# TensorHusker/Butterfly

Hardware: AMD Instinct MI355X
Metric: tokens/sec (node) + p50 latency, Llama-3-70B split across 1/2/4/8 MI355X (higher is better)
Workload: dtype bf16; 1 GPU; model=Llama-3-70B, global_batch=64, seq_len=1024, parallelism=single, hipgraph=True, kv_cache_dtype=bfloat16, async_decode=True, mixed=True, prefix_caching=True

## Files before the change

### butterfly_amd/ops/__init__.py

```python
from __future__ import annotations

import os
import threading
from typing import Optional
from pathlib import Path

import torch

from . import reference as ref
from .reference import SILU_INTERLEAVE, interleave_gate_up, rope_tables, split_gate_up

_LIB_PATH = Path(__file__).resolve().parent.parent / "_C.so"
_loaded = False
_load_error: str | None = None

EPILOGUES = {"none": 0, "bias": 1, "silu": 2}
DECODE_PART_TOKENS = 0


def load_library(path: str | os.PathLike | None = None) -> bool:
    global _loaded, _load_error
    if _loaded:
        return True
    p = Path(path) if path else Path(os.environ.get("BFLY_KERNEL_LIB") or _LIB_PATH)
# ... 528 lines not shown
        torch.ops.bfly.w8_scale_cols(y, scale, out, epi)
    return out


def linear_silu_gate(x, w, gates, e0: int, num_local: int, packed=None):
    if isinstance(x, RowNormed) or not _gpu(x):
        h = linear(x, w, epilogue="silu")
        return moe_gate_scale_(h, gates, e0, num_local)
    out = _empty(x.shape[0], w.shape[0] // 2, dtype=x.dtype, device=x.device)
    if packed is not None and torch.ops.bfly.gemm_packed(x, packed, out, 3, None, 0.0, gates, e0, num_local) > 0:
        return out
    torch.ops.bfly.gemm_silu_gate(x, w, out, gates, e0, num_local)
    return out


def gemm_plan(M: int, N: int, K: int) -> dict:
    load_library()
    k, mt, nt, bm, bn, sk, wk = torch.ops.bfly.gemm_plan(M, N, K)
    return {"kind": ("skinny", "tile", "big", "dec", "big8", "mid8", "big4", "mid4")[k], "mt": mt, "nt": nt, "wk": wk, "bm": bm, "bn": bn,
            "splitk": sk}


def attn_prefill(q, k, v, cu_seqlens, max_seqlen: int, scale: float, causal: bool = True,
                 out=None, cu_seqlens_k=None, return_lse: bool = False):
    if not _gpu(q):
        return ref.attn_prefill(q, k, v, cu_seqlens, max_seqlen, scale, causal, out, cu_seqlens_k, return_lse)
    if out is None:
        out = _empty(q.shape, dtype=q.dtype, device=q.device)
    lse = _empty(q.shape[0], q.shape[1], dtype=torch.float32, device=q.device) if return_lse else None
    torch.ops.bfly.attn_prefill(q, k, v, cu_seqlens, max_seqlen, scale, causal, out, cu_seqlens_k, lse)
    return (out, lse) if return_lse else out


def attn_prefill_paged(q, k_cache, v_cache, tables, cu_q, positions, max_q: int, scale: float, out=None):
    if not _gpu(q):
# ... 136 lines not shown
```

### butterfly_amd/utils/flags.py

```python
from __future__ import annotations

import os
from dataclasses import dataclass
from typing import Any, Callable


@dataclass(frozen=True)
class Flag:
    name: str
    default: Any
    parse: Callable[[str], Any]
    help: str


def _bool(s: str) -> bool:
    return s.strip().lower() in ("1", "true", "yes", "on")


FLAGS: dict[str, Flag] = {}


def define(name: str, default, parse, help: str) -> Flag:
    f = Flag(name, default, parse, help)
    FLAGS[name] = f
# ... 12 lines not shown
define("BFLY_CUSTOM_AR", True, _bool, "use the one-shot IPC all-reduce kernel (self-tested at start-up, "
       "RCCL otherwise) for small TP all-reduces")
define("BFLY_CUSTOM_AR_MAX_BYTES", 8 << 20, int, "largest all-reduce (bytes) routed to the IPC kernel")
define("BFLY_CUSTOM_AR_AUTOTUNE", True, _bool, "time the IPC all-reduce (one- / two-shot) against RCCL at start-up "
       "and route each message size to the faster one (0: the fixed BFLY_CUSTOM_AR_* thresholds)")
define("BFLY_AR_BUTTERFLY", "", str, "\"W@lo:hi[,...]\": all-reduces of lo..hi bytes over a group of W ranks (bare "
       "\"lo:hi\": any power-of-two group) run as the butterfly "
       "(recursive halving + doubling over point-to-point transfers, parallel/butterfly.py), outside graph capture; set by "
       "the start-up probe only where it measured faster than RCCL and the IPC kernel (empty = never)")
define("BFLY_PROBE_BUTTERFLY", False, _bool, "the start-up comm probe also times the butterfly all-reduce (and may "
       "route sizes to it through BFLY_AR_BUTTERFLY)")
define("BFLY_CUSTOM_AR_2SHOT_BYTES", 512 << 10, int, "IPC all-reduces of at least this many bytes over 4 or 8 "
       "ranks run as reduce-scatter + all-gather (2S/W bytes per link instead of S; 0 = always one-shot)")
define("BFLY_GEMM_TUNED", True, _bool, "consult the measured GEMM plan table (0: heuristic plans only; read by the kernel library)")
define("BFLY_GEMM_NT_WEIGHTS", True, _bool, "stream decode GEMM weights with the non-temporal policy (read by the kernel library)")
define("BFLY_GEMM_PLAN", "", str, "force GEMM plans for whole-model A/B runs: \"N,K,Mbucket:kind,mt,nt,wk,bm,bn,sk;...\" "
       "(read by the kernel library)")
define("BFLY_ATTN_XCD", 1, int, "prefill attention: XCD-aware item walk (0: plain order; read by the kernel library)")
define("BFLY_ATTN_TRACE", "", str, "set: the prefill attention kernel stamps its item phases into the LSE buffer "
       "instead of writing results (tools/attn_trace.py; read by the kernel library)")
define("BFLY_KERNEL_LIB", "", str, "path of another build of the kernel library (same-box A/B runs of kernel changes)")
define("BFLY_LOG_JSON", False, _bool, "emit log records as one JSON object per line")
define("BFLY_RESTART", 0, int, "restart attempt of this job (set by `launch --max-restarts`; 0 = first run)")
define("BFLY_ATTN_PAGED_LDS", True, _bool, "paged-prefix prefill attention: the LDS-staged kernel for chunks of "
       "several sequences (0: the register kernel everywhere; read by the kernel library)")
define("BFLY_DEFER_REDUCE", True, _bool, "fuse split-K GEMM reduces into the consuming rope / add+rmsnorm kernels")
define("BFLY_NORM_ROWSCALE", True, _bool, "decode add+RMSNorm split over (row, 1024-column) workgroups that write x * g "
       "and partial sums of squares; the consuming QKV / gate-up GEMM applies the 1/rms row scale in its epilogue "
       "(tp == 1, batches <= BFLY_NORM_ROWSCALE_MAX_ROWS; 0: one-workgroup-per-row add+RMSNorm)")
define("BFLY_NORM_ROWSCALE_MAX_ROWS", 256, int, "largest batch that takes the row-split add+RMSNorm")
# ... 83 lines not shown
```

### csrc/bindings/ops.cpp

```cpp
#include <ATen/ATen.h>
#include <ATen/hip/impl/HIPStreamMasqueradingAsCUDA.h>
#include <c10/core/DeviceGuard.h>
#include <torch/library.h>

#include "bfly_kernels.h"

namespace {

using at::Tensor;

inline hipStream_t cur_stream() { return at::hip::getCurrentHIPStreamMasqueradingAsCUDA().stream(); }

inline bfly::bf16* bf(const Tensor& t) { return reinterpret_cast<bfly::bf16*>(t.data_ptr()); }

#define CHECK_GPU(t) TORCH_CHECK((t).is_cuda(), #t " must be a GPU tensor")
#define CHECK_BF16(t) TORCH_CHECK((t).scalar_type() == at::kBFloat16, #t " must be bf16")
#define CHECK_INNER(t) TORCH_CHECK((t).stride(-1) == 1, #t " must have unit inner stride")
#define CHECK_ALIGN16(t) \
  TORCH_CHECK(reinterpret_cast<uintptr_t>((t).data_ptr()) % 16 == 0, #t " must be 16-B aligned")
#define CHECK_KV(k, v)                                                                          \
  TORCH_CHECK(((k).scalar_type() == at::kBFloat16 || (k).scalar_type() == at::kFloat8_e4m3fn) && \
                  (v).scalar_type() == (k).scalar_type(),                                       \
              "KV caches must both be bf16 or both float8_e4m3fn")
#define CHECK_I32(t) TORCH_CHECK((t).scalar_type() == at::kInt, #t " must be int32")
// ... 517 lines not shown
    ws = workspace->data_ptr<float>();
    ws_bytes = workspace->numel() * sizeof(float);
  }
  c10::DeviceGuard g(x.device());
  const int rc = bfly::launch_gemm_w8(bf(x), x.stride(0), u8(code), scale.data_ptr<float>(), M, N, K, (int)epilogue,
                                      bf(out), out.stride(0), ws, ws_bytes, cur_stream(), any_m, (int)force_sk);
  TORCH_CHECK(rc == 0, "gemm_w8: shape / plan not taken by the native kernel M=", M, " N=", N, " K=", K,
              " (rc=", rc, ")");
}

int64_t gemm_packed_check(int64_t M, int64_t N, int64_t K, int64_t epilogue) {
  return bfly::launch_gemm_packed(nullptr, 0, nullptr, (int)M, (int)N, (int)K, (int)epilogue, nullptr, 0, nullptr,
                                  nullptr, true);
}

void gemm_with_plan(const Tensor& x, const Tensor& w, Tensor& out, std::vector<int64_t> plan,
                    int64_t epilogue, const c10::optional<Tensor>& workspace,
                    const c10::optional<Tensor>& bias) {
  CHECK_GPU(x); CHECK_BF16(x); CHECK_BF16(w); CHECK_BF16(out);
  TORCH_CHECK(x.dim() == 2 && w.dim() == 2 && out.dim() == 2 && plan.size() == 7, "gemm_with_plan: args");
  CHECK_INNER(x); CHECK_INNER(w); CHECK_INNER(out);
  const int M = x.size(0), K = x.size(1), N = w.size(0);
  TORCH_CHECK(w.size(1) == K, "gemm_with_plan: K mismatch");
  const int nout = epilogue == bfly::EPI_SILU ? N / 2 : N;
  TORCH_CHECK(out.size(0) == M && out.size(1) == nout, "gemm_with_plan: out shape");
  bfly::GemmPlan p{};
  p.kind = plan[0]; p.mt = plan[1]; p.nt = plan[2]; p.wk = plan[3]; p.bm = plan[4]; p.bn = plan[5]; p.sk = plan[6];
  float* ws = nullptr;
  size_t ws_bytes = 0;
  if (workspace.has_value()) {
    ws = reinterpret_cast<float*>(workspace->data_ptr());
    ws_bytes = workspace->numel() * workspace->element_size();
  }
  const bfly::bf16* bp = nullptr;
  if (bias.has_value()) {
    TORCH_CHECK(epilogue == bfly::EPI_BIAS && bias->numel() == N && bias->is_contiguous(), "gemm_with_plan: bias");
    CHECK_BF16(*bias);
    bp = bf(*bias);
  }
  TORCH_CHECK(epilogue != bfly::EPI_BIAS || bp != nullptr, "gemm_with_plan: bias epilogue needs a bias");
  c10::DeviceGuard g(x.device());
  const int rc = bfly::launch_gemm_plan(p, bf(x), x.stride(0), bf(w), w.stride(0), M, N, K, epilogue,
                                        bp, bf(out), out.stride(0), ws, ws_bytes, cur_stream());
  TORCH_CHECK(rc == 0, "gemm_with_plan: plan rejected (rc=", rc, ")");
}

int64_t gemm_deferred(const Tensor& x, const Tensor& w, Tensor& out, Tensor& workspace) {
  CHECK_GPU(x); CHECK_BF16(x); CHECK_BF16(w); CHECK_BF16(out);
  TORCH_CHECK(x.dim() == 2 && w.dim() == 2 && out.dim() == 2, "gemm_deferred: 2-D operands");
  CHECK_INNER(x); CHECK_INNER(w); CHECK_INNER(out);
  CHECK_ALIGN16(x); CHECK_ALIGN16(w);
  const int M = x.size(0), K = x.size(1), N = w.size(0);
  TORCH_CHECK(w.size(1) == K && K % 64 == 0 && N % 128 == 0, "gemm_deferred: shape");
  TORCH_CHECK(x.stride(0) % 8 == 0 && w.stride(0) % 8 == 0, "gemm_deferred: row strides % 8");
  TORCH_CHECK(out.size(0) == M && out.size(1) == N && out.is_contiguous(), "gemm_deferred: out");
  TORCH_CHECK(workspace.scalar_type() == at::kFloat && workspace.is_contiguous(), "gemm_deferred: workspace");
  c10::DeviceGuard g(x.device());
  const int rc = bfly::launch_gemm_deferred(bf(x), x.stride(0), bf(w), w.stride(0), M, N, K, bf(out),
// ... 663 lines not shown
  m.def("gemm_packed(Tensor x, Tensor wp, Tensor(a!) out, int epilogue, Tensor? ssp=None, float eps=0.0, "
        "Tensor? gates=None, int e0=0, int num_local=1, Tensor(b!)? workspace=None, bool defer=False) -> int");
  m.def("gemm_packed_check(int M, int N, int K, int epilogue) -> int", &gemm_packed_check);
  m.def("quant_fp8_rows(Tensor w, Tensor(a!) code, Tensor(b!) scale) -> ()");
  m.def("dequant_fp8(Tensor code, Tensor? scale, Tensor(a!) out) -> ()");
  m.def("w8_scale_cols(Tensor y, Tensor scale, Tensor(a!) out, int epilogue) -> ()");
  m.def("gemm_w8(Tensor x, Tensor code, Tensor scale, Tensor(a!) out, int epilogue, Tensor(b!)? workspace, "
        "bool any_m=False, int force_sk=0) -> ()");
  m.def("gemm_w8_check(int M, int N, int K, int epilogue) -> int",
        [](int64_t M, int64_t N, int64_t K, int64_t e) -> int64_t { return bfly::gemm_w8_check(M, N, K, e); });
  m.def("gemm_w8_splitk(int M, int N, int K, int epilogue) -> int",
        [](int64_t M, int64_t N, int64_t K, int64_t e) -> int64_t { return bfly::gemm_w8_splitk(M, N, K, e); });
  m.def("gemm_w8_workspace_size(int M, int N, int K) -> int",
        [](int64_t M, int64_t N, int64_t K) -> int64_t { return (int64_t)bfly::gemm_w8_workspace_bytes(M, N, K); });
  m.def("gemm_with_plan(Tensor x, Tensor w, Tensor(a!) out, int[] plan, int epilogue, Tensor(b!)? workspace, "
        "Tensor? bias=None) -> ()");
  m.def("gemm_workspace_size(int M, int N, int K) -> int", &gemm_workspace_size);
  m.def("gemm_plan(int M, int N, int K) -> int[]", &gemm_plan);
  m.def("gemm_check(int M, int N, int K, int epilogue) -> int",
        [](int64_t M, int64_t N, int64_t K, int64_t e) -> int64_t { return bfly::gemm_check(M, N, K, e); });
  m.def("attn_decode_splits(int max_ctx, int part_tokens) -> int", &attn_decode_splits);
  m.def("attn_decode_part_tokens(int B, int Hkv, int max_ctx) -> int", &attn_decode_part_tokens);
  m.def("attn_decode(Tensor q, Tensor k_cache, Tensor v_cache, Tensor block_tables, Tensor ctx_lens, "
        "float scale, int max_ctx, int part_tokens, Tensor(a!) out, Tensor(b!)? part_o, "
        "Tensor(c!)? part_ml) -> ()");
  m.def("moe_route(Tensor x, Tensor wr, int top_k, Tensor(a!) gates, Tensor(b!) topk_ids, Tensor(c!) topk_w) -> ()");
  m.def("moe_gate_scale(Tensor(a!) h, Tensor gates, int e0, int num_local) -> ()");
  m.def("moe_max_tiles(int tk, int num_local, int bm=64) -> int", &moe_max_tiles);
  m.def("moe_align(Tensor topk_ids, int e0, int num_local, Tensor(a!) rows, Tensor(b!) slot_of, Tensor(c!) tiles, "
        "Tensor(d!) count, int bm=64, Tensor? bcnt=None, int bcap=0) -> ()");
  m.def("moe_grouped_gemm(Tensor x, Tensor w, Tensor(a!) out, Tensor? rows, Tensor tiles, Tensor count, int w_estride, "
// ... 99 lines not shown
```

### csrc/include/bfly_kernels.h

```cpp
#pragma once
#include <hip/hip_runtime.h>
#include <stddef.h>
#include <stdint.h>

namespace bfly {

typedef __bf16 bf16;

enum GemmEpilogue { EPI_NONE = 0, EPI_BIAS = 1, EPI_SILU = 2, EPI_SILU_GATE = 3 };

struct RowScale {
  const float* ss;
  int chunks;
  float inv_dim, eps;
  const float* gate = nullptr;
  int gld = 0, ge0 = 0, gF = 0;
};

struct GemmPlan {
  int kind;
  int mt, nt;
  int wk;
  int bm, bn;
  int sk;
// ... 51 lines not shown
constexpr int kLogprobsMaxChunks = 64;
inline int logprobs_chunks(int V) { return (V + kLogprobsChunk - 1) / kLogprobsChunk; }
inline size_t logprobs_workspace_words(long rows, int V, int n) {
  return (size_t)rows * logprobs_chunks(V) * (2 + n);
}
void launch_logprobs_partial(const bf16* logits, long row_stride, int rows, int V, int vstart,
                             const int* ids, int n, uint64_t* workspace, float* record,
                             hipStream_t stream);
void launch_logprobs_merge(const float* records, int tp, int rows, int n, float* chosen_lp,
                           int* top_ids, float* top_lp, hipStream_t stream);

GemmPlan plan_gemm(int M, int N, int K);
size_t gemm_workspace_bytes(int M, int N, int K);
int launch_gemm_plan(const GemmPlan& p, const bf16* X, long ldx, const bf16* W, long ldw, int M,
                     int N, int K, int epi, const bf16* bias, bf16* out, long ldo, float* ws,
                     size_t ws_bytes, hipStream_t stream);
int gemm_check(int M, int N, int K, int epi);
int gemm_rowscale_check(int M, int N, int K, int epi);
int launch_gemm_deferred(const bf16* X, long ldx, const bf16* W, long ldw, int M, int N, int K,
                         bf16* out, long ldo, float* ws, size_t ws_bytes, hipStream_t stream,
                         const RowScale* rs = nullptr);
size_t gemm_slab_offset_floats();
void launch_splitk_reduce(const float* part, int sk, int M, int N, bf16* out, long ldo,
                          hipStream_t stream);
int launch_gemm(const bf16* X, long ldx, const bf16* W, long ldw, int M, int N, int K, int epi,
                const bf16* bias, bf16* out, long ldo, float* ws, size_t ws_bytes,
                hipStream_t stream, const RowScale* rs = nullptr);
int launch_gemm_packed(const bf16* X, long ldx, const bf16* Wp, int M, int N, int K, int epi, bf16* out,
                       long ldo, hipStream_t stream, const RowScale* rs = nullptr, bool dry = false,
                       float* ws = nullptr, size_t ws_bytes = 0, bool defer = false);
int launch_gemm_silu_gate(const bf16* X, long ldx, const bf16* W, long ldw, int M, int N, int K,
// ... 101 lines not shown
```

### csrc/kernels/gemm.hip

```cpp
#include "bfly_common.h"

#include <cstdio>
#include <string>
#include <vector>
#include "bfly_kernels.h"
#include "bfly_kv.h"

namespace bfly {

typedef __attribute__((address_space(3))) void* lds_ptr_t;

__constant__ int g_tile_w_nt = 1;
typedef __attribute__((address_space(1))) void* gbl_ptr_t;

__device__ __forceinline__ void store_out(bf16* out, long ldo, int m, int n, float v) {
  out[(long)m * ldo + n] = f2bf(v);
}

__device__ __forceinline__ void store_out4(bf16* out, long ldo, int m, int n, f32x4 v, bool vec) {
  bf16* p = out + (long)m * ldo + n;
  if (vec) {
    bf16x4 o;
#pragma unroll
    for (int r = 0; r < 4; ++r) o[r] = f2bf(v[r]);
// ... 183 lines not shown
    else
      __builtin_amdgcn_global_load_lds((gbl_ptr_t)g, (lds_ptr_t)(lds + blk * 1024), 16, 0, 0);
  }
}

template <int N>
__device__ __forceinline__ void vm_wait() {
  asm volatile("s_waitcnt vmcnt(%0)" ::"n"(N) : "memory");
}

__device__ __forceinline__ bf16x8 lds_frag(const char* lds, int row, int chunk) {
  const int slot = chunk ^ ((row >> 1) & 7);
  return *reinterpret_cast<const bf16x8*>(lds + row * 128 + slot * 16);
}

template <int TI, int TJ>
__device__ __forceinline__ void tile_epilogue(const f32x4 (&acc)[TI][TJ], int mw, int nw, int lane,
                                              int M, int N, int epi, const bf16* __restrict__ bias,
                                              bf16* __restrict__ out, long ldo, float* __restrict__ pslab,
                                              int m0, const RowScale& rsc) {
  const int lr = lane & 15, lc = 4 * (lane >> 4);
  const auto rs = slab_rsrc(pslab, pslab ? (long)(M - m0) * N * 4 : 0);
  const bool vec = (ldo & 3) == 0 && (reinterpret_cast<uintptr_t>(out) & 7) == 0;
  float sc[TI];
#pragma unroll
  for (int i = 0; i < TI; ++i) sc[i] = 1.f;
  if (rsc.ss != nullptr) {
    const int q = lane >> 4, nc = rsc.chunks;
#pragma unroll
    for (int i = 0; i < TI; ++i) {
      const int m = min(mw + 16 * i + lr, M - 1);
// ... 14 lines not shown
    }
  }
#pragma unroll
  for (int i = 0; i < TI; ++i) {
    const int m = mw + 16 * i + lr;
    if (m >= M) continue;
#pragma unroll
    for (int j = 0; j < TJ; ++j) {
      const int n = nw + 16 * j + lc;
      if (pslab) {
        store_slab4(rs, ((m - m0) * N + n) * 4, acc[i][j] * sc[i]);
      } else if (epi == EPI_SILU || epi == EPI_SILU_GATE) {
        if constexpr (TJ % 2 == 0) {
          if (j & 1) continue;
          f32x4 h;
#pragma unroll
          for (int r = 0; r < 4; ++r) h[r] = silu(acc[i][j][r] * sc[i]) * (acc[i][j + 1][r] * sc[i]);
          const int f = nw / 2 + 16 * (j / 2) + lc;
          if (epi == EPI_SILU_GATE) {
            const float g = rsc.gate[(long)m * rsc.gld + rsc.ge0 + f / rsc.gF];
#pragma unroll
            for (int r = 0; r < 4; ++r) h[r] = bf2f(f2bf(h[r])) * g;
          }
          store_out4(out, ldo, m, f, h, vec);
        }
      } else {
        f32x4 v = acc[i][j] * sc[i];
        if (epi == EPI_BIAS) {
#pragma unroll
          for (int r = 0; r < 4; ++r) v[r] += bf2f(bias[n + r]);
        }
        store_out4(out, ldo, m, n, v, vec);
// ... 82 lines not shown
    for (int ks = 0; ks < 2; ++ks) {
      bf16x8 af[TI], bfr[TJ];
#pragma unroll
      for (int i = 0; i < TI; ++i) af[i] = lds_frag(As, wm * WM + 16 * i + (lane & 15), ks * 4 + (lane >> 4));
#pragma unroll
      for (int j = 0; j < TJ; ++j) bfr[j] = lds_frag(Bs, wn * WN + 16 * j + (lane & 15), ks * 4 + (lane >> 4));
#pragma unroll
      for (int i = 0; i < TI; ++i)
#pragma unroll
        for (int j = 0; j < TJ; ++j) acc[i][j] = mfma16(bfr[j], af[i], acc[i][j]);
    }
    if (++buf == STAGES) buf = 0;
  }
  tile_epilogue<TI, TJ>(acc, m0 + wm * WM, n0 + wn * WN, lane, M, N, epi, bias, out, ldo,
                        part ? part + (long)ksplit * m_slab * N + (long)m0 * N : nullptr, m0, rsc);
}

template <int ROWS, int NW>
constexpr int ring_loads() { return (ROWS / 8 + NW - 1) / NW; }

template <int ROWS, int NW>
__device__ __forceinline__ void ring_stage(const bf16* __restrict__ src, long ld, int row0, int row_max,
                                           int k0, char* lds, int wid, int lane, bool nt) {
  constexpr int kBlocks = ROWS / 8;
#pragma unroll
  for (int i = 0; i < ring_loads<ROWS, NW>(); ++i) {
    int blk = i * NW + wid;
    if (kBlocks % NW != 0) blk %= kBlocks;
    const int row = blk * 8 + (lane >> 3);
    const int chunk = (lane & 7) ^ ((row >> 1) & 7);
// ... 772 lines not shown
  init_nt_policy();
  const int tiles = ((M + BM - 1) / BM) * (N / BN);
  const size_t lds = (size_t)STAGES * (BM + BN) * kBK * 2;
  const dim3 grid(tiles, sk);
  static bool attr_set = false;
  if (!attr_set && lds > 65536) {
    hipFuncSetAttribute(reinterpret_cast<const void*>(&gemm_tile_kernel<BM, BN, WMW, STAGES, false, PACKW>),
                        hipFuncAttributeMaxDynamicSharedMemorySize, (int)lds);
    attr_set = true;
  }
  gemm_tile_kernel<BM, BN, WMW, STAGES, false, PACKW><<<grid, kTileThreads, lds, stream>>>(
      X, ldx, W, PACKW ? (long)K : ldw, M, N, K, epi, bias, out, ldo, sk > 1 ? splitk_part(ws) : nullptr,
      nullptr, nullptr, nullptr, 0, rsc);
}

template <int BM, int BN, int NWM, int NWN, int SW>
static void run_dec(const bf16* X, long ldx, const bf16* W, long ldw, int M, int N, int K,
                    int epi, const bf16* bias, bf16* out, long ldo, float* ws, int sk,
                    hipStream_t stream, const RowScale& rsc) {
  init_nt_policy();
  const int tiles = ((M + BM - 1) / BM) * (N / BN);
  constexpr size_t lds = (size_t)(3 * BM + SW * BN) * kBK * 2;
  static_assert(lds <= 160 * 1024, "decode GEMM rings exceed the 160 KiB LDS");
  static bool attr_set = false;
  if (!attr_set && lds > 65536) {
    hipFuncSetAttribute(reinterpret_cast<const void*>(&gemm_dec_kernel<BM, BN, NWM, NWN, SW>),
                        hipFuncAttributeMaxDynamicSharedMemorySize, (int)lds);
    attr_set = true;
  }
  const dim3 grid(tiles, sk);
// ... 87 lines not shown
    size_t pos = 0;
    while (pos < s.size()) {
      size_t end = s.find(';', pos);
      if (end == std::string::npos) end = s.size();
      PlanOverride o{};
      if (sscanf(s.substr(pos, end - pos).c_str(), "%d,%d,%d:%d,%d,%d,%d,%d,%d,%d", &o.N, &o.K, &o.M, &o.p.kind,
                 &o.p.mt, &o.p.nt, &o.p.wk, &o.p.bm, &o.p.bn, &o.p.sk) == 10)
        out.push_back(o);
      pos = end + 1;
    }
    return out;
  }();
  return v;
}

GemmPlan plan_gemm(int M, int N, int K) {
  if (!plan_overrides().empty()) {
    static const int kB[] = {1, 16, 32, 64, 128, 256, 512};
    int bucket = 0;
    for (int b : kB)
      if (b >= M) { bucket = b; break; }
    for (const PlanOverride& o : plan_overrides())
      if (o.N == N && o.K == K && o.M == bucket) return o.p;
  }
  if (!tuned_enabled()) return plan_gemm_heuristic(M, N, K);
  static const int kBuckets[] = {1, 16, 32, 64, 128, 256, 512};
  int bucket = 0;
  for (int b : kBuckets)
    if (b >= M) { bucket = b; break; }
  if (bucket == 0) return plan_gemm_heuristic(M, N, K);
  for (const TunedPlan& t : kTuned)
    if (t.N == N && t.K == K && t.M == bucket)
      return t.kind == 4 ? GemmPlan{6, 0, 0, 0, 256, 256, t.sk}
                         : GemmPlan{t.kind, t.mt, t.nt, t.wk, t.bm, t.bn, t.sk};
  return plan_gemm_heuristic(M, N, K);
}

static GemmPlan plan_gemm_heuristic(int M, int N, int K) {
  GemmPlan p{};
  const int target = 448;
  const bool skinny_ok = K % 128 == 0 && N % 128 == 0;
  if (skinny_ok && (M <= 4 || (M <= 64 && K <= 1024))) {
    p.kind = 0;
    p.mt = (M + 15) / 16;
    const bool long_k = K > 4096;
    p.nt = M <= 4 ? (long_k ? 4 : 2) : 2;
    p.wk = long_k ? 2 : 4;
    const int blocks = N / (16 * p.nt * (4 / p.wk));
    int sk = 1;
    const int nchunks = K / 128;
// ... 29 lines not shown
static size_t plan_ws_bytes(const GemmPlan& p, int M, int N) {
  return p.sk > 1 ? kCounterBytes + (size_t)p.sk * M * N * sizeof(float) : 0;
}

size_t gemm_workspace_bytes(int M, int N, int K) {
  const size_t a = plan_ws_bytes(plan_gemm(M, N, K), M, N);
  const size_t b = plan_ws_bytes(plan_gemm_heuristic(M, N, K), M, N);
  return a > b ? a : b;
}

static int run_plan(const GemmPlan& p, const bf16* X, long ldx, const bf16* W, long ldw, int M,
                    int N, int K, int epi, const bf16* bias, bf16* out, long ldo, float* ws,
                    hipStream_t stream, bool dry = false, bool defer = false,
                    const RowScale* rs = nullptr, bool packed = false) {
  const RowScale rsc = rs ? *rs : RowScale{nullptr, 0, 0.f, 0.f};
  if (rs != nullptr && p.kind != 1 && p.kind != 3 && p.kind != 5 && p.kind != 7) return -4;
  if (epi == EPI_SILU_GATE && (p.kind != 1 || p.sk != 1)) return -4;
  if (packed && p.kind != 5 && p.kind != 7) return -5;
  if (p.kind == 4) {
    if (N % 256 != 0 || K % 64 != 0 || K / 64 < 2 * p.sk) return -1;
    if (!dry) run_big8(X, ldx, W, ldw, M, N, K, epi, bias, out, ldo, ws, p.sk, stream);
  } else if (p.kind == 7) {
    if (N % p.bn != 0 || K % 64 != 0 || K / 64 < p.sk) return -1;
    bool done = false;
#define MID4_CASE(BM_, BN_, SA_, SB_)                                                               \
  if (!done && p.bm == BM_ && p.bn == BN_ && p.mt == SA_ && p.nt == SB_) {                          \
    if (!dry && packed) run_mid4<BM_, BN_, SA_, SB_, true>(X, ldx, W, ldw, M, N, K, epi, bias, out, ldo, ws, p.sk, stream, rsc); \
    else if (!dry) run_mid4<BM_, BN_, SA_, SB_>(X, ldx, W, ldw, M, N, K, epi, bias, out, ldo, ws, p.sk, stream, rsc); \
    done = true;                                                                                   \
  }
    MID4_CASE(128, 128, 4, 6) MID4_CASE(128, 128, 3, 7) MID4_CASE(128, 128, 2, 8)
    MID4_CASE(256, 128, 3, 4) MID4_CASE(256, 128, 2, 6) MID4_CASE(128, 256, 4, 3) MID4_CASE(128, 256, 2, 4)
#undef MID4_CASE
// ... 41 lines not shown
    if (N % (16 * p.nt * (4 / p.wk)) != 0) return -1;
    if (epi == EPI_SILU && p.nt % 2 != 0) return -1;
    if (p.sk > 1 && N / (16 * p.nt * (4 / p.wk)) > kSplitCounters) return -1;
    bool done = false;
#define SK_CASE(MT_, NT_, WK_)                                                                   \
  if (!done && p.mt == MT_ && p.nt == NT_ && p.wk == WK_) {                                       \
    if (!dry) run_skinny<MT_, NT_, WK_>(X, ldx, W, ldw, M, N, K, epi, bias, out, ldo, ws, p.sk, stream); \
    done = true;                                                                                  \
  }
#define SK_WK(MT_, NT_) SK_CASE(MT_, NT_, 1) SK_CASE(MT_, NT_, 2) SK_CASE(MT_, NT_, 4)
    SK_WK(1, 1) SK_WK(1, 2) SK_WK(1, 4) SK_WK(2, 1) SK_WK(2, 2) SK_WK(2, 4)
    SK_WK(3, 2) SK_WK(4, 1) SK_WK(4, 2) SK_WK(4, 4)
#undef SK_WK
#undef SK_CASE
    if (!done) return -2;
  } else if (p.kind == 1 && p.nt == 1) {
    if (N % 256 != 0 || K % 64 != 0 || (p.bm != 16 && p.bm != 32 && p.bm != 64) || (p.bn != 128 && p.bn != 256) ||
        K / kBK < p.sk)
      return -1;
    if (p.sk > 1 && (long)((M + p.bm - 1) / p.bm) * (N / p.bn) > kSplitCounters) return -1;
    bool done = false;
    const int st = p.mt > 0 ? p.mt : 2;
#define TLP_CASE(BM_, BN_, WMW_, ST_)                                                                 \
  if (!done && p.bm == BM_ && p.bn == BN_ && p.wk == WMW_ && st == ST_) {                             \
    if (!dry) run_tile<BM_, BN_, WMW_, ST_, true>(X, ldx, W, ldw, M, N, K, epi, bias, out, ldo, ws, p.sk, stream, rsc); \
    done = true;                                                                                      \
  }
#define TLP_ST(BM_, BN_, WMW_) TLP_CASE(BM_, BN_, WMW_, 2) TLP_CASE(BM_, BN_, WMW_, 3) TLP_CASE(BM_, BN_, WMW_, 4)
    TLP_ST(16, 128, 1) TLP_ST(16, 256, 1) TLP_ST(32, 128, 1) TLP_ST(32, 256, 1)
    TLP_ST(64, 128, 1) TLP_ST(64, 128, 2) TLP_ST(64, 256, 1) TLP_ST(64, 256, 2)
#undef TLP_ST
// ... 19 lines not shown
    if (!done) return -2;
  }
  if (p.sk > 1 && !dry && !defer) {
    const int nout = epi == EPI_SILU ? N / 2 : N;
    long total = (long)M * nout;
    int grid = (int)((total + 255) / 256);
    if (grid > 4096) grid = 4096;
    gemm_splitk_reduce_kernel<<<grid, 256, 0, stream>>>(splitk_part(ws), p.sk, M, N, epi, bias,
                                                         out, ldo);
  }
  return 0;
}

int launch_gemm_plan(const GemmPlan& p, const bf16* X, long ldx, const bf16* W, long ldw, int M,
                     int N, int K, int epi, const bf16* bias, bf16* out, long ldo, float* ws,
                     size_t ws_bytes, hipStream_t stream) {
  if (M <= 0) return 0;
  if (p.sk > 1 && (ws == nullptr || ws_bytes < kCounterBytes + (size_t)p.sk * M * N * sizeof(float)))
    return -3;
  return run_plan(p, X, ldx, W, ldw, M, N, K, epi, bias, out, ldo, ws, stream);
}

static GemmPlan select_plan(int M, int N, int K, int epi) {
  GemmPlan p = plan_gemm(M, N, K);
  if (run_plan(p, nullptr, 0, nullptr, 0, M, N, K, epi, nullptr, nullptr, 0, nullptr, nullptr, true) != 0)
    p = plan_gemm_heuristic(M, N, K);
  return p;
}

int gemm_rowscale_check(int M, int N, int K, int epi) {
  if (M <= 0) return 0;
  const RowScale probe{nullptr, 0, 0.f, 0.f};
  return run_plan(select_plan(M, N, K, epi), nullptr, 0, nullptr, 0, M, N, K, epi, nullptr, nullptr, 0,
                  nullptr, nullptr, true, false, &probe);
}
// ... 84 lines not shown
}

int launch_gemm(const bf16* X, long ldx, const bf16* W, long ldw, int M, int N, int K, int epi,
                const bf16* bias, bf16* out, long ldo, float* ws, size_t ws_bytes,
                hipStream_t stream, const RowScale* rs) {
  if (M <= 0) return 0;
  GemmPlan p = select_plan(M, N, K, epi);
  if (p.sk > 1 && (ws == nullptr || ws_bytes < kCounterBytes + (size_t)p.sk * M * N * sizeof(float)))
    p.sk = 1;
  return run_plan(p, X, ldx, W, ldw, M, N, K, epi, bias, out, ldo, ws, stream, false, false, rs);
}

struct PackedTuned { int N, K, M; GemmPlan p; };
static const PackedTuned kPackedTuned[] = {
    {8192, 8192, 64, {1, 3, 1, 2, 64, 128, 4}},
    {4096, 4096, 1, {-1, 0, 0, 0, 0, 0, 0}},
    {4096, 4096, 16, {-1, 0, 0, 0, 0, 0, 0}},
    {4096, 4096, 32, {-1, 0, 0, 0, 0, 0, 0}},
    {4096, 4096, 64, {-1, 0, 0, 0, 0, 0, 0}},
};

int launch_gemm_packed(const bf16* X, long ldx, const bf16* Wp, int M, int N, int K, int epi, bf16* out,
                       long ldo, hipStream_t stream, const RowScale* rs, bool dry, float* ws, size_t ws_bytes,
                       bool defer) {
  if (M <= 0) return dry ? 0 : 1;
  if (N % 256 != 0 || K % 64 != 0) return -1;
  GemmPlan p = plan_gemm(M, N, K);
  if (tuned_enabled() && plan_overrides().empty() && epi != EPI_SILU_GATE) {
    static const int kB[] = {1, 16, 32, 64, 128, 256, 512};
    int bucket = 0;
    for (int b : kB)
      if (b >= M) { bucket = b; break; }
    for (const PackedTuned& t : kPackedTuned)
      if (t.N == N && t.K == K && t.M == bucket) {
        if (t.p.kind < 0) return -2;
        if (run_plan(t.p, nullptr, 0, nullptr, 0, M, N, K, epi, nullptr, nullptr, 0, nullptr, nullptr, true) == 0)
          p = t.p;
        break;
      }
  }
  if (epi != EPI_SILU_GATE &&
      run_plan(p, nullptr, 0, nullptr, 0, M, N, K, epi, nullptr, nullptr, 0, nullptr, nullptr, true) != 0)
    p = plan_gemm_heuristic(M, N, K);
  if (epi == EPI_SILU_GATE &&
      run_plan(p, nullptr, 0, nullptr, 0, M, N, K, epi, nullptr, nullptr, 0, nullptr, nullptr, true) != 0) {
    const int bm = M <= 16 ? 16 : M <= 32 ? 32 : M <= 64 ? 64 : 128;
    p = GemmPlan{1, 3, 0, bm <= 32 ? 1 : 2, bm, 128, 1};
  }
  const bool mid = (p.kind == 5 || p.kind == 7) && (p.bn == 128 || p.bn == 256);
  if (!mid && (p.kind != 1 || (p.bm != 16 && p.bm != 32 && p.bm != 64) || (p.bn != 128 && p.bn != 256))) return -2;
  if (!dry && p.sk > 1 && (ws == nullptr || ws_bytes < kCounterBytes + (size_t)p.sk * M * N * sizeof(float)))
    return -3;
  if (!mid) p.nt = 1;
  if (dry)
    return run_plan(p, nullptr, 0, nullptr, 0, M, N, K, epi, nullptr, nullptr, 0, nullptr, nullptr, true, false,
                    nullptr, mid);
  const bool d = defer && p.sk > 1;
  const int rc = run_plan(p, X, ldx, Wp, K, M, N, K, epi, nullptr, out, ldo, ws, stream, false, d, rs, mid);
  if (rc != 0) return rc;
  return d ? p.sk : 1;
}

int launch_gemm_silu_gate(const bf16* X, long ldx, const bf16* W, long ldw, int M, int N, int K,
                          bf16* out, long ldo, const float* gates, int gld, int ge0, int gF,
                          hipStream_t stream) {
  if (M <= 0) return 0;
  if (gates == nullptr || gF <= 0 || gF % 16 != 0 || (N / 2) % gF != 0) return -5;
  GemmPlan p = plan_gemm(M, N, K);
  if (run_plan(p, nullptr, 0, nullptr, 0, M, N, K, EPI_SILU_GATE, nullptr, nullptr, 0, nullptr, nullptr, true) != 0) {
    const int bm = M <= 16 ? 16 : M <= 32 ? 32 : M <= 64 ? 64 : 128;
    p = GemmPlan{1, 3, 0, bm <= 32 ? 1 : 2, bm, 128, 1};
  }
  RowScale rs{nullptr, 0, 0.f, 0.f};
// ... 9 lines not shown
```

Measured before the change: 2253 tokens/s.

## Add mixed-width (128+96) column tile GEMM kernel to balance decode CU load

Measured after the change: 2300 tokens/s, median of 6. 2.1% higher.

```diff
diff --git a/butterfly_amd/ops/__init__.py b/butterfly_amd/ops/__init__.py
--- a/butterfly_amd/ops/__init__.py
+++ b/butterfly_amd/ops/__init__.py
@@ -566,11 +566,13 @@
     return out
 
 
+GEMM_KINDS = ("skinny", "tile", "big", "dec", "big8", "mid8", "big4", "mid4", "mixed")
+
+
 def gemm_plan(M: int, N: int, K: int) -> dict:
     load_library()
     k, mt, nt, bm, bn, sk, wk = torch.ops.bfly.gemm_plan(M, N, K)
-    return {"kind": ("skinny", "tile", "big", "dec", "big8", "mid8", "big4", "mid4")[k], "mt": mt, "nt": nt, "wk": wk, "bm": bm, "bn": bn,
-            "splitk": sk}
+    return {"kind": GEMM_KINDS[k], "mt": mt, "nt": nt, "wk": wk, "bm": bm, "bn": bn, "splitk": sk}
 
 
 def attn_prefill(q, k, v, cu_seqlens, max_seqlen: int, scale: float, causal: bool = True,
diff --git a/butterfly_amd/utils/flags.py b/butterfly_amd/utils/flags.py
--- a/butterfly_amd/utils/flags.py
+++ b/butterfly_amd/utils/flags.py
@@ -50,6 +50,9 @@
        "ranks run as reduce-scatter + all-gather (2S/W bytes per link instead of S; 0 = always one-shot)")
 define("BFLY_GEMM_TUNED", True, _bool, "consult the measured GEMM plan table (0: heuristic plans only; read by the kernel library)")
 define("BFLY_GEMM_NT_WEIGHTS", True, _bool, "stream decode GEMM weights with the non-temporal policy (read by the kernel library)")
+define("BFLY_GEMM_MIXED_TILES", 1, int, "decode GEMM column tiles of two widths (128 + 96) in one launch, so every CU "
+       "carries the same columns: 0 = never, 1 = the measured shapes on their packed weight (gemm.hip kPackedTuned), "
+       "2 = every decode tile plan whose N splits (read by the kernel library)")
 define("BFLY_GEMM_PLAN", "", str, "force GEMM plans for whole-model A/B runs: \"N,K,Mbucket:kind,mt,nt,wk,bm,bn,sk;...\" "
        "(read by the kernel library)")
 define("BFLY_ATTN_XCD", 1, int, "prefill attention: XCD-aware item walk (0: plain order; read by the kernel library)")
diff --git a/csrc/bindings/ops.cpp b/csrc/bindings/ops.cpp
--- a/csrc/bindings/ops.cpp
+++ b/csrc/bindings/ops.cpp
@@ -555,14 +555,22 @@
                                   nullptr, true);
 }
 
+int64_t gemm_plan_check(std::vector<int64_t> plan, int64_t M, int64_t N, int64_t K, int64_t epilogue, bool packed) {
+  TORCH_CHECK(plan.size() == 7, "gemm_plan_check: plan");
+  bfly::GemmPlan p{};
+  p.kind = plan[0]; p.mt = plan[1]; p.nt = plan[2]; p.wk = plan[3]; p.bm = plan[4]; p.bn = plan[5]; p.sk = plan[6];
+  return bfly::gemm_plan_check(p, (int)M, (int)N, (int)K, (int)epilogue, packed);
+}
+
 void gemm_with_plan(const Tensor& x, const Tensor& w, Tensor& out, std::vector<int64_t> plan,
                     int64_t epilogue, const c10::optional<Tensor>& workspace,
-                    const c10::optional<Tensor>& bias) {
+                    const c10::optional<Tensor>& bias, bool packed) {
   CHECK_GPU(x); CHECK_BF16(x); CHECK_BF16(w); CHECK_BF16(out);
   TORCH_CHECK(x.dim() == 2 && w.dim() == 2 && out.dim() == 2 && plan.size() == 7, "gemm_with_plan: args");
   CHECK_INNER(x); CHECK_INNER(w); CHECK_INNER(out);
   const int M = x.size(0), K = x.size(1), N = w.size(0);
   TORCH_CHECK(w.size(1) == K, "gemm_with_plan: K mismatch");
+  TORCH_CHECK(!packed || (w.is_contiguous() && N % 256 == 0 && K % 64 == 0), "gemm_with_plan: packed weight");
   const int nout = epilogue == bfly::EPI_SILU ? N / 2 : N;
   TORCH_CHECK(out.size(0) == M && out.size(1) == nout, "gemm_with_plan: out shape");
   bfly::GemmPlan p{};
@@ -582,7 +590,7 @@
   TORCH_CHECK(epilogue != bfly::EPI_BIAS || bp != nullptr, "gemm_with_plan: bias epilogue needs a bias");
   c10::DeviceGuard g(x.device());
   const int rc = bfly::launch_gemm_plan(p, bf(x), x.stride(0), bf(w), w.stride(0), M, N, K, epilogue,
-                                        bp, bf(out), out.stride(0), ws, ws_bytes, cur_stream());
+                                        bp, bf(out), out.stride(0), ws, ws_bytes, cur_stream(), packed);
   TORCH_CHECK(rc == 0, "gemm_with_plan: plan rejected (rc=", rc, ")");
 }
 
@@ -1276,7 +1284,10 @@
   m.def("gemm_w8_workspace_size(int M, int N, int K) -> int",
         [](int64_t M, int64_t N, int64_t K) -> int64_t { return (int64_t)bfly::gemm_w8_workspace_bytes(M, N, K); });
   m.def("gemm_with_plan(Tensor x, Tensor w, Tensor(a!) out, int[] plan, int epilogue, Tensor(b!)? workspace, "
-        "Tensor? bias=None) -> ()");
+        "Tensor? bias=None, bool packed=False) -> ()");
+  m.def("gemm_plan_check(int[] plan, int M, int N, int K, int epilogue, bool packed=False) -> int", &gemm_plan_check);
+  m.def("gemm_mixed_tiles_mode(int mode) -> int",
+        [](int64_t mode) -> int64_t { return bfly::gemm_mixed_tiles_mode((int)mode); });
   m.def("gemm_workspace_size(int M, int N, int K) -> int", &gemm_workspace_size);
   m.def("gemm_plan(int M, int N, int K) -> int[]", &gemm_plan);
   m.def("gemm_check(int M, int N, int K, int epilogue) -> int",
diff --git a/csrc/include/bfly_kernels.h b/csrc/include/bfly_kernels.h
--- a/csrc/include/bfly_kernels.h
+++ b/csrc/include/bfly_kernels.h
@@ -89,7 +89,9 @@
 size_t gemm_workspace_bytes(int M, int N, int K);
 int launch_gemm_plan(const GemmPlan& p, const bf16* X, long ldx, const bf16* W, long ldw, int M,
                      int N, int K, int epi, const bf16* bias, bf16* out, long ldo, float* ws,
-                     size_t ws_bytes, hipStream_t stream);
+                     size_t ws_bytes, hipStream_t stream, bool packed = false);
+int gemm_plan_check(const GemmPlan& p, int M, int N, int K, int epi, bool packed);
+int gemm_mixed_tiles_mode(int mode);
 int gemm_check(int M, int N, int K, int epi);
 int gemm_rowscale_check(int M, int N, int K, int epi);
 int launch_gemm_deferred(const bf16* X, long ldx, const bf16* W, long ldw, int M, int N, int K,
diff --git a/csrc/kernels/gemm.hip b/csrc/kernels/gemm.hip
--- a/csrc/kernels/gemm.hip
+++ b/csrc/kernels/gemm.hip
@@ -221,7 +221,7 @@
   return *reinterpret_cast<const bf16x8*>(lds + row * 128 + slot * 16);
 }
 
-template <int TI, int TJ>
+template <int TI, int TJ, int SFORM = 0>
 __device__ __forceinline__ void tile_epilogue(const f32x4 (&acc)[TI][TJ], int mw, int nw, int lane,
                                               int M, int N, int epi, const bf16* __restrict__ bias,
                                               bf16* __restrict__ out, long ldo, float* __restrict__ pslab,
@@ -266,8 +266,19 @@
         if constexpr (TJ % 2 == 0) {
           if (j & 1) continue;
           f32x4 h;
-#pragma unroll
-          for (int r = 0; r < 4; ++r) h[r] = silu(acc[i][j][r] * sc[i]) * (acc[i][j + 1][r] * sc[i]);
+          if constexpr (SFORM != 0) {
+#pragma clang fp reassociate(off) contract(off)
+            const float s = sc[i], s2 = s * s, c = -1.44269504f * s;
+#pragma unroll
+            for (int r = 0; r < 4; ++r) {
+              const float g = acc[i][j][r], u = acc[i][j + 1][r];
+              const float rcp = __builtin_amdgcn_rcpf(__builtin_amdgcn_exp2f(g * c) + 1.f);
+              h[r] = (SFORM == 1 ? (s2 * g) * u : s2 * (g * u)) * rcp;
+            }
+          } else {
+#pragma unroll
+            for (int r = 0; r < 4; ++r) h[r] = silu(acc[i][j][r] * sc[i]) * (acc[i][j + 1][r] * sc[i]);
+          }
           const int f = nw / 2 + 16 * (j / 2) + lc;
           if (epi == EPI_SILU_GATE) {
             const float g = rsc.gate[(long)m * rsc.gld + rsc.ge0 + f / rsc.gF];
@@ -380,6 +391,105 @@
   }
   tile_epilogue<TI, TJ>(acc, m0 + wm * WM, n0 + wn * WN, lane, M, N, epi, bias, out, ldo,
                         part ? part + (long)ksplit * m_slab * N + (long)m0 * N : nullptr, m0, rsc);
+}
+
+template <int BM, int BN, int WMW, int STAGES, bool PACKW, int SFORM>
+__device__ __forceinline__ void tile_body(const bf16* __restrict__ X, long ldx, const bf16* __restrict__ W,
+                                          long ldw, int M, int N, int K, int epi,
+                                          const bf16* __restrict__ bias, bf16* __restrict__ out, long ldo,
+                                          float* __restrict__ part, int m0, int n0, const RowScale& rsc,
+                                          char* smem) {
+  constexpr int WNW = 4 / WMW;
+  constexpr int WM = BM / WMW;
+  constexpr int WN = BN % (16 * WNW) == 0 ? BN / WNW : 32;
+  constexpr int NACT = BN / WN;
+  static_assert(BN % WN == 0 && NACT <= WNW && WM % 16 == 0 && WN % 16 == 0, "wave layout");
+  constexpr int TI = WM / 16, TJ = WN / 16;
+  constexpr int A_BYTES = BM * kBK * 2, B_BYTES = BN * kBK * 2;
+  constexpr int LPW = stage_loads<BM>() + stage_loads<BN>();
+  constexpr int STAGE_BYTES = A_BYTES + B_BYTES;
+
+  const int lane = threadIdx.x & 63, wid = threadIdx.x >> 6;
+  const int wm = wid / WNW, wn = wid % WNW;
+  const bool active = NACT == WNW || wn < NACT;
+  const int ksplit = (int)blockIdx.y;
+  const int nsplit = (int)gridDim.y;
+
+  const int ktiles = K / kBK;
+  const int kt0 = (int)(((long)ktiles * ksplit) / nsplit);
+  const int kt1 = (int)(((long)ktiles * (ksplit + 1)) / nsplit);
+  const bool w_nt = M <= BM && g_tile_w_nt;
+
+  f32x4 acc[TI][TJ];
+#pragma unroll
+  for (int i = 0; i < TI; ++i)
+#pragma unroll
+    for (int j = 0; j < TJ; ++j) acc[i][j] = f32x4{0.f, 0.f, 0.f, 0.f};
+
+#pragma unroll
+  for (int s = 0; s < STAGES - 1; ++s) {
+    if (kt0 + s < kt1) {
+      char* b = smem + s * STAGE_BYTES;
+      tile_stage<BM>(X, ldx, m0, M, (kt0 + s) * kBK, b, wid, lane);
+      tile_stage<BN, false, PACKW>(W, ldw, n0, N, (kt0 + s) * kBK, b + A_BYTES, wid, lane, nullptr, w_nt);
+    }
+  }
+  int buf = 0;
+  for (int kt = kt0; kt < kt1; ++kt) {
+    const int after = min(STAGES - 2, kt1 - 1 - kt);
+    if (STAGES >= 4 && after >= 2) vm_wait<(STAGES >= 4 ? 2 : 0) * LPW>();
+    else if (STAGES >= 3 && after >= 1) vm_wait<LPW>();
+    else vm_wait<0>();
+    asm volatile("s_waitcnt lgkmcnt(0)" ::: "memory");
+    __builtin_amdgcn_s_barrier();
+    if (kt + STAGES - 1 < kt1) {
+      int nbuf = buf + STAGES - 1;
+      if (nbuf >= STAGES) nbuf -= STAGES;
+      char* nb = smem + nbuf * STAGE_BYTES;
+      tile_stage<BM>(X, ldx, m0, M, (kt + STAGES - 1) * kBK, nb, wid, lane);
+      tile_stage<BN, false, PACKW>(W, ldw, n0, N, (kt + STAGES - 1) * kBK, nb + A_BYTES, wid, lane, nullptr, w_nt);
+    }
+    const char* As = smem + buf * STAGE_BYTES;
+    const char* Bs = As + A_BYTES;
+    if (active) {
+#pragma unroll
+      for (int ks = 0; ks < 2; ++ks) {
+        bf16x8 af[TI], bfr[TJ];
+#pragma unroll
+        for (int i = 0; i < TI; ++i) af[i] = lds_frag(As, wm * WM + 16 * i + (lane & 15), ks * 4 + (lane >> 4));
+#pragma unroll
+        for (int j = 0; j < TJ; ++j) bfr[j] = lds_frag(Bs, wn * WN + 16 * j + (lane & 15), ks * 4 + (lane >> 4));
+#pragma unroll
+        for (int i = 0; i < TI; ++i)
+#pragma unroll
+          for (int j = 0; j < TJ; ++j) acc[i][j] = mfma16(bfr[j], af[i], acc[i][j]);
+      }
+    }
+    if (++buf == STAGES) buf = 0;
+  }
+  if (active)
+    tile_epilogue<TI, TJ, SFORM>(acc, m0 + wm * WM, n0 + wn * WN, lane, M, N, epi, bias, out, ldo,
+                                 part ? part + (long)ksplit * M * N + (long)m0 * N : nullptr, m0, rsc);
+}
+
+template <int BM, int BNW, int WMWW, int BNN, int WMWN, int STAGES, bool PACKW>
+__global__ void __launch_bounds__(kTileThreads)
+gemm_tile_mixed_kernel(const bf16* __restrict__ X, long ldx, const bf16* __restrict__ W, long ldw,
+                       int M, int N, int K, int epi, const bf16* __restrict__ bias,
+                       bf16* __restrict__ out, long ldo, float* __restrict__ part, int nwide, RowScale rsc) {
+  extern __shared__ __attribute__((aligned(16))) char smem[];
+  constexpr int SFORM = BM == 16 ? 2 : 1;
+  const int mtiles = (M + BM - 1) / BM;
+  const int wide_wgs = nwide * mtiles, b = (int)blockIdx.x;
+  if (b < wide_wgs) {
+    const int tile = xcd_remap(b, wide_wgs);
+    tile_body<BM, BNW, WMWW, STAGES, PACKW, SFORM>(X, ldx, W, ldw, M, N, K, epi, bias, out, ldo, part,
+                                                   (tile % mtiles) * BM, (tile / mtiles) * BNW, rsc, smem);
+  } else {
+    const int tile = xcd_remap(b - wide_wgs, (int)gridDim.x - wide_wgs);
+    tile_body<BM, BNN, WMWN, STAGES, PACKW, SFORM>(X, ldx, W, ldw, M, N, K, epi, bias, out, ldo, part,
+                                                   (tile % mtiles) * BM, nwide * BNW + (tile / mtiles) * BNN, rsc, smem);
+  }
 }
 
 template <int ROWS, int NW>
@@ -1182,6 +1292,26 @@
       nullptr, nullptr, nullptr, 0, rsc);
 }
 
+template <int BM, int BNW, int WMWW, int BNN, int WMWN, int STAGES, bool PACKW>
+static void run_tile_mixed(const bf16* X, long ldx, const bf16* W, long ldw, int M, int N, int K,
+                           int epi, const bf16* bias, bf16* out, long ldo, float* ws, int sk,
+                           hipStream_t stream, const RowScale& rsc, int nwide, int nnarrow) {
+  init_nt_policy();
+  const int mtiles = (M + BM - 1) / BM;
+  const size_t lds = (size_t)STAGES * (BM + BNW) * kBK * 2;
+  const dim3 grid((nwide + nnarrow) * mtiles, sk);
+  static bool attr_set = false;
+  if (!attr_set && lds > 65536) {
+    hipFuncSetAttribute(
+        reinterpret_cast<const void*>(&gemm_tile_mixed_kernel<BM, BNW, WMWW, BNN, WMWN, STAGES, PACKW>),
+        hipFuncAttributeMaxDynamicSharedMemorySize, (int)lds);
+    attr_set = true;
+  }
+  gemm_tile_mixed_kernel<BM, BNW, WMWW, BNN, WMWN, STAGES, PACKW><<<grid, kTileThreads, lds, stream>>>(
+      X, ldx, W, PACKW ? (long)K : ldw, M, N, K, epi, bias, out, ldo, sk > 1 ? splitk_part(ws) : nullptr, nwide,
+      rsc);
+}
+
 template <int BM, int BN, int NWM, int NWN, int SW>
 static void run_dec(const bf16* X, long ldx, const bf16* W, long ldw, int M, int N, int K,
                     int epi, const bf16* bias, bf16* out, long ldo, float* ws, int sk,
@@ -1299,26 +1429,40 @@
   return v;
 }
 
+constexpr int kMixedWide = 128, kMixedNarrow = 96;
+static int g_mixed_mode = -1;
+
+int gemm_mixed_tiles_mode(int mode) {
+  if (g_mixed_mode < 0) {
+    const char* e = getenv("BFLY_GEMM_MIXED_TILES");
+    g_mixed_mode = e && e[0] >= '0' && e[0] <= '2' ? e[0] - '0' : 1;
+  }
+  const int prev = g_mixed_mode;
+  if (mode >= 0 && mode <= 2) g_mixed_mode = mode;
+  return prev;
+}
+
+static GemmPlan mixed_plan(const GemmPlan& p, int N) {
+  if (gemm_mixed_tiles_mode(-1) != 2 || p.kind != 1 || p.nt != 0 || p.bn != kMixedWide || p.bm > 64 || p.mt != 3 ||
+      N % (kMixedWide + kMixedNarrow) != 0)
+    return p;
+  return GemmPlan{8, 3, 0, kMixedNarrow, p.bm, kMixedWide, p.sk};
+}
+
 GemmPlan plan_gemm(int M, int N, int K) {
-  if (!plan_overrides().empty()) {
-    static const int kB[] = {1, 16, 32, 64, 128, 256, 512};
-    int bucket = 0;
-    for (int b : kB)
-      if (b >= M) { bucket = b; break; }
-    for (const PlanOverride& o : plan_overrides())
-      if (o.N == N && o.K == K && o.M == bucket) return o.p;
-  }
-  if (!tuned_enabled()) return plan_gemm_heuristic(M, N, K);
   static const int kBuckets[] = {1, 16, 32, 64, 128, 256, 512};
   int bucket = 0;
   for (int b : kBuckets)
     if (b >= M) { bucket = b; break; }
+  for (const PlanOverride& o : plan_overrides())
+    if (o.N == N && o.K == K && o.M == bucket) return o.p;
+  if (!tuned_enabled()) return mixed_plan(plan_gemm_heuristic(M, N, K), N);
   if (bucket == 0) return plan_gemm_heuristic(M, N, K);
   for (const TunedPlan& t : kTuned)
     if (t.N == N && t.K == K && t.M == bucket)
       return t.kind == 4 ? GemmPlan{6, 0, 0, 0, 256, 256, t.sk}
                          : GemmPlan{t.kind, t.mt, t.nt, t.wk, t.bm, t.bn, t.sk};
-  return plan_gemm_heuristic(M, N, K);
+  return mixed_plan(plan_gemm_heuristic(M, N, K), N);
 }
 
 static GemmPlan plan_gemm_heuristic(int M, int N, int K) {
@@ -1378,9 +1522,9 @@
                     hipStream_t stream, bool dry = false, bool defer = false,
                     const RowScale* rs = nullptr, bool packed = false) {
   const RowScale rsc = rs ? *rs : RowScale{nullptr, 0, 0.f, 0.f};
-  if (rs != nullptr && p.kind != 1 && p.kind != 3 && p.kind != 5 && p.kind != 7) return -4;
-  if (epi == EPI_SILU_GATE && (p.kind != 1 || p.sk != 1)) return -4;
-  if (packed && p.kind != 5 && p.kind != 7) return -5;
+  if (rs != nullptr && p.kind != 1 && p.kind != 3 && p.kind != 5 && p.kind != 7 && p.kind != 8) return -4;
+  if (epi == EPI_SILU_GATE && ((p.kind != 1 && p.kind != 8) || p.sk != 1)) return -4;
+  if (packed && p.kind != 1 && p.kind != 5 && p.kind != 7 && p.kind != 8) return -5;
   if (p.kind == 4) {
     if (N % 256 != 0 || K % 64 != 0 || K / 64 < 2 * p.sk) return -1;
     if (!dry) run_big8(X, ldx, W, ldw, M, N, K, epi, bias, out, ldo, ws, p.sk, stream);
@@ -1452,7 +1596,29 @@
 #undef SK_WK
 #undef SK_CASE
     if (!done) return -2;
-  } else if (p.kind == 1 && p.nt == 1) {
+  } else if (p.kind == 8) {
+    if (p.bn != kMixedWide || p.wk != kMixedNarrow || N % (p.bn + p.wk) != 0 || K % kBK != 0 || K / kBK < p.sk ||
+        p.sk < 1 || (packed && N % 256 != 0))
+      return -1;
+    if ((epi == EPI_SILU || epi == EPI_SILU_GATE) && (p.bn % 32 != 0 || p.wk % 32 != 0)) return -1;
+    const int npair = N / (p.bn + p.wk);
+    if (p.sk > 1 && 2L * npair * ((M + p.bm - 1) / p.bm) > kSplitCounters) return -1;
+    bool done = false;
+    const int st = p.mt > 0 ? p.mt : 3;
+#define MX_CASE(BM_, WMWW_, WMWN_)                                                                    \
+  if (!done && p.bm == BM_ && st == 3) {                                                              \
+    if (!dry && packed)                                                                               \
+      run_tile_mixed<BM_, kMixedWide, WMWW_, kMixedNarrow, WMWN_, 3, true>(X, ldx, W, ldw, M, N, K, epi, bias, out, \
+                                                                           ldo, ws, p.sk, stream, rsc, npair, npair); \
+    else if (!dry)                                                                                    \
+      run_tile_mixed<BM_, kMixedWide, WMWW_, kMixedNarrow, WMWN_, 3, false>(X, ldx, W, ldw, M, N, K, epi, bias, out, \
+                                                                            ldo, ws, p.sk, stream, rsc, npair, npair); \
+    done = true;                                                                                      \
+  }
+    MX_CASE(16, 1, 1) MX_CASE(32, 1, 1) MX_CASE(64, 2, 4)
+#undef MX_CASE
+    if (!done) return -2;
+  } else if (p.kind == 1 && packed) {
     if (N % 256 != 0 || K % 64 != 0 || (p.bm != 16 && p.bm != 32 && p.bm != 64) || (p.bn != 128 && p.bn != 256) ||
         K / kBK < p.sk)
       return -1;
@@ -1502,11 +1668,17 @@
 
 int launch_gemm_plan(const GemmPlan& p, const bf16* X, long ldx, const bf16* W, long ldw, int M,
                      int N, int K, int epi, const bf16* bias, bf16* out, long ldo, float* ws,
-                     size_t ws_bytes, hipStream_t stream) {
+                     size_t ws_bytes, hipStream_t stream, bool packed) {
   if (M <= 0) return 0;
   if (p.sk > 1 && (ws == nullptr || ws_bytes < kCounterBytes + (size_t)p.sk * M * N * sizeof(float)))
     return -3;
-  return run_plan(p, X, ldx, W, ldw, M, N, K, epi, bias, out, ldo, ws, stream);
+  return run_plan(p, X, ldx, W, packed ? (long)K : ldw, M, N, K, epi, bias, out, ldo, ws, stream, false, false,
+                  nullptr, packed);
+}
+
+int gemm_plan_check(const GemmPlan& p, int M, int N, int K, int epi, bool packed) {
+  return run_plan(p, nullptr, 0, nullptr, 0, M, N, K, epi, nullptr, nullptr, 0, nullptr, nullptr, true, false,
+                  nullptr, packed);
 }
 
 static GemmPlan select_plan(int M, int N, int K, int epi) {
@@ -1621,6 +1793,7 @@
 struct PackedTuned { int N, K, M; GemmPlan p; };
 static const PackedTuned kPackedTuned[] = {
     {8192, 8192, 64, {1, 3, 1, 2, 64, 128, 4}},
+    {57344, 8192, 64, {8, 3, 0, kMixedNarrow, 64, kMixedWide, 1}},
     {4096, 4096, 1, {-1, 0, 0, 0, 0, 0, 0}},
     {4096, 4096, 16, {-1, 0, 0, 0, 0, 0, 0}},
     {4096, 4096, 32, {-1, 0, 0, 0, 0, 0, 0}},
@@ -1641,6 +1814,7 @@
     for (const PackedTuned& t : kPackedTuned)
       if (t.N == N && t.K == K && t.M == bucket) {
         if (t.p.kind < 0) return -2;
+        if (t.p.kind == 8 && gemm_mixed_tiles_mode(-1) == 0) break;
         if (run_plan(t.p, nullptr, 0, nullptr, 0, M, N, K, epi, nullptr, nullptr, 0, nullptr, nullptr, true) == 0)
           p = t.p;
         break;
@@ -1655,15 +1829,15 @@
     p = GemmPlan{1, 3, 0, bm <= 32 ? 1 : 2, bm, 128, 1};
   }
   const bool mid = (p.kind == 5 || p.kind == 7) && (p.bn == 128 || p.bn == 256);
-  if (!mid && (p.kind != 1 || (p.bm != 16 && p.bm != 32 && p.bm != 64) || (p.bn != 128 && p.bn != 256))) return -2;
+  const bool tile = (p.kind == 1 && (p.bn == 128 || p.bn == 256)) || p.kind == 8;
+  if (!mid && (!tile || (p.bm != 16 && p.bm != 32 && p.bm != 64))) return -2;
   if (!dry && p.sk > 1 && (ws == nullptr || ws_bytes < kCounterBytes + (size_t)p.sk * M * N * sizeof(float)))
     return -3;
-  if (!mid) p.nt = 1;
   if (dry)
     return run_plan(p, nullptr, 0, nullptr, 0, M, N, K, epi, nullptr, nullptr, 0, nullptr, nullptr, true, false,
-                    nullptr, mid);
+                    nullptr, true);
   const bool d = defer && p.sk > 1;
-  const int rc = run_plan(p, X, ldx, Wp, K, M, N, K, epi, nullptr, out, ldo, ws, stream, false, d, rs, mid);
+  const int rc = run_plan(p, X, ldx, Wp, K, M, N, K, epi, nullptr, out, ldo, ws, stream, false, d, rs, true);
   if (rc != 0) return rc;
   return d ? p.sk : 1;
 }
```
